# MikeWangWZHL/VidIL

Hardware: AMD Instinct MI355X
Metric: frames/sec whole-node (BLIP caption+filt + CLIP visual-token) 224^2 8f/video (higher is better)
Workload: dtype bf16

## Files before the change

### vidil_amd/csrc/attention.hip

```cpp
#include <type_traits>

#include "common.h"
#include "gemm_epilogue.h"

namespace {

template <typename T>
struct AttnP {
  const T* q;
  const T* k;
  const T* vt;
  T* out;
  const int32_t* kv_len;
  const int32_t* kv_index;
  const int32_t* group_start;
  int Bq, H, Nq, Nk, Tq_cap, Tk_cap, NP, kv_group, causal, causal_off, ldo, n_kv;
  int out_mode;
  int tiled;
  int rb;
  int ostage;
  const float* q32;
  long long ldq32;
  float q_scale;
};
// ... 551 lines not shown
#pragma unroll
      for (int kt = KA - 1; kt < NKT; ++kt) issue_half(uu, kt, 4);
    };
    issue_first(u);
    for (;;) {
      asm volatile("s_waitcnt vmcnt(0)" ::: "memory");
      __builtin_amdgcn_s_barrier();
      issue_second(u);
      asm volatile("s_waitcnt vmcnt(0)" ::: "memory");
      __builtin_amdgcn_s_barrier();
      u += stride;
      if (u >= nunits) break;
      issue_first(u);
    }
    return;
  }

  const int hi = lane >> 5, l31 = lane & 31;
  const int sw = (l31 >> 1) & 7;
  const int row = wave * 32 + l31;
  const bool valid = row < p.Nq;
  const int vc = valid ? row : p.Nq - 1;
  const int vlane = ((lane >> 4) & 1) * VSUB + (hi * 4 + ((lane & 15) >> 2)) * 32 + (lane & 3) * 8;
  char* scratch = smem + NKT * TILE + wave * 2048;
  f16x8 qf[4];
  const uint32_t q_off = (uint32_t)(vc * 128 + hi * 16);
  const __amdgpu_buffer_rsrc_t rsrc_q = uniform_rsrc(p.q, (uint32_t)nunits * p.Tq_cap * 128);
  auto load_q = [&](int uu, f16x8 (&dst)[4]) {
    const uint32_t ub = (uint32_t)uu * p.Tq_cap * 128;
#pragma unroll
    for (int ks = 0; ks < 4; ++ks)
      dst[ks] = __builtin_bit_cast(f16x8, __builtin_amdgcn_raw_buffer_load_b128(rsrc_q, q_off + ks * 32, ub, 0));
  };
  const uint32_t row_off = valid ? (uint32_t)row * p.ldo * (OUT8 ? 1 : 2) : 0x80000000u;
  load_q(u, qf);
  asm volatile("" ::"v"(qf[0]), "v"(qf[1]), "v"(qf[2]), "v"(qf[3]));
  auto read_k2 = [&](int kt, int h2, f16x8 (&kf)[2]) {
    const char* ks_ = smem + kt * TILE + l31 * 128;
#pragma unroll
    for (int j = 0; j < 2; ++j) kf[j] = *(const f16x8*)(ks_ + ((((h2 * 2 + j) * 2 + hi) ^ sw) << 4));
  };
  auto read_v2 = [&](int kt, int hb, f16x8 (&vf)[2]) {
    const char* vs_ = smem + kt * TILE + 4096 + vlane + hb * 512;
#pragma unroll
    for (int dt = 0; dt < 2; ++dt) {
      const char* a = vs_ + dt * (2 * VSUB);
      const s16x4 lo = __builtin_amdgcn_ds_read_tr16_b64_v4i16((__attribute__((address_space(3))) s16x4*)(a));
      const s16x4 hi4 = __builtin_amdgcn_ds_read_tr16_b64_v4i16((__attribute__((address_space(3))) s16x4*)(a + 256));
      typedef short s16x8 __attribute__((ext_vector_type(8)));
      const s16x8 both = __builtin_shufflevector(lo, hi4, 0, 1, 2, 3, 4, 5, 6, 7);
      vf[dt] = __builtin_bit_cast(f16x8, both);
    }
  };
  const f32x16 zero16 = {0.f, 0.f, 0.f, 0.f, 0.f, 0.f, 0.f, 0.f, 0.f, 0.f, 0.f, 0.f, 0.f, 0.f, 0.f, 0.f};
#ifndef VIDIL_ATTN_QAHEAD
#define VIDIL_ATTN_QAHEAD 2
#endif
  constexpr int QAHEAD = VIDIL_ATTN_QAHEAD;
  f16x8 qn[4];
#ifdef VIDIL_ATTN_TIMING
  uint64_t t_b1 = 0, t_b2 = 0, t_st = 0;
  const uint64_t t_begin = __builtin_amdgcn_s_memtime();
#endif
  for (;;) {
    float m, l;
    f32x16 O[2], S;
    f16x8 pf[2];
#ifdef VIDIL_ATTN_TIMING
    const uint64_t tb1 = __builtin_amdgcn_s_memtime();
#endif
    __builtin_amdgcn_s_barrier();
    asm volatile("" ::: "memory");
#ifdef VIDIL_ATTN_TIMING
    t_b1 += __builtin_amdgcn_s_memtime() - tb1;
#endif
    auto fused = [&](int kt, auto first_tag) {
      constexpr bool FIRST = decltype(first_tag)::value;
      f16x8 kf[2], vf[2];
#ifdef VIDIL_ATTN_PRIO
      __builtin_amdgcn_s_setprio(VIDIL_ATTN_PRIO);
#endif
#pragma unroll
      for (int hb = 0; hb < 2; ++hb) {
        read_v2(kt, hb, vf);
        read_k2(kt + 1, hb, kf);
        O[0] = Elt<T>::mfma32(vf[0], pf[hb], FIRST && hb == 0 ? zero16 : O[0]);
        S = Elt<T>::mfma32(kf[0], qf[hb * 2], hb == 0 ? zero16 : S);
        O[1] = Elt<T>::mfma32(vf[1], pf[hb], FIRST && hb == 0 ? zero16 : O[1]);
        S = Elt<T>::mfma32(kf[1], qf[hb * 2 + 1], S);
        __builtin_amdgcn_sched_barrier(0);
      }
#ifdef VIDIL_ATTN_PRIO
      __builtin_amdgcn_s_setprio(0);
#endif
    };
    {
      f16x8 kf[2];
      read_k2(0, 0, kf);
      S = Elt<T>::mfma32(kf[0], qf[0], zero16);
      S = Elt<T>::mfma32(kf[1], qf[1], S);
      read_k2(0, 1, kf);
      S = Elt<T>::mfma32(kf[0], qf[2], S);
      S = Elt<T>::mfma32(kf[1], qf[3], S);
    }
    softmax_tile<T, false, true>(S, 0, nk, false, m, l, O, pf);
    fused(0, std::true_type{});
#pragma unroll 1
    for (int kt = 1; kt < NKT - 1; ++kt) {
      if (kt == QAHEAD) load_q(u + stride < nunits ? u + stride : u, qn);
      softmax_tile<T, false>(S, kt * 32, nk, false, m, l, O, pf);
#ifdef VIDIL_ATTN_TIMING
      const uint64_t tb2 = __builtin_amdgcn_s_memtime();
#endif
      if (kt == KA - 1) __builtin_amdgcn_s_barrier();
      asm volatile("" ::: "memory");
#ifdef VIDIL_ATTN_TIMING
      if (kt == KA - 1) t_b2 += __builtin_amdgcn_s_memtime() - tb2;
#endif
      fused(kt, std::false_type{});
    }
    const int un = u + stride;
    const int bk = u / p.H, h = u - bk * p.H;
#pragma unroll
    for (int ks = 0; ks < 4; ++ks) qf[ks] = qn[ks];
    softmax_tile<T, true>(S, (NKT - 1) * 32, nk, true, m, l, O, pf);
#pragma unroll
    for (int hb = 0; hb < 2; ++hb) {
      f16x8 vf[2];
      read_v2(NKT - 1, hb, vf);
      O[0] = Elt<T>::mfma32(vf[0], pf[hb], O[0]);
      O[1] = Elt<T>::mfma32(vf[1], pf[hb], O[1]);
    }
    l += __shfl_xor(l, 32, 64);
    const float inv = l > 0.f ? 1.0f / l : 0.f;
#ifdef VIDIL_ATTN_TIMING
    const uint64_t ts0 = __builtin_amdgcn_s_memtime();
#endif
#if defined(VIDIL_ATTN_ABLATE) && (VIDIL_ATTN_ABLATE & 2)
    if (inv == 12345.f)
#endif
    {
      if constexpr (OUT8) {
        const __amdgpu_buffer_rsrc_t rsrc = uniform_rsrc((const char*)p.out + ((size_t)bk * p.Nq * p.ldo + h * 64), (uint32_t)p.Nq * p.ldo);
        store_rows_stream_fp8(rsrc, row_off, O, inv, scratch);
      } else {
        const __amdgpu_buffer_rsrc_t rsrc = uniform_rsrc(p.out + ((size_t)bk * p.Nq * p.ldo + h * 64), (uint32_t)p.Nq * p.ldo * 2);
        store_rows_stream<T>(rsrc, row_off, O, inv, scratch);
      }
    }
#ifdef VIDIL_ATTN_TIMING
    t_st += __builtin_amdgcn_s_memtime() - ts0;
#endif
    if (un >= nunits) break;
    u = un;
  }
#ifdef VIDIL_ATTN_TIMING
  if (lane == 0) {
    asm volatile("s_waitcnt vmcnt(0)" ::: "memory");
    uint64_t* dbg = (uint64_t*)p.out + ((size_t)blockIdx.x * 8 + wave) * 4;
    dbg[0] = __builtin_amdgcn_s_memtime() - t_begin;
    dbg[1] = t_b1;
    dbg[2] = t_b2;
    dbg[3] = t_st;
  }
#endif
}

template <typename T, bool QS, int D, bool TILED>
__global__ __launch_bounds__(256, (QS || !TILED) ? 2 : 3) void attn_direct1_kernel(const AttnP<T> p) {
  using f16 = T;
  using f16x8 = typename Elt<T>::x8;
  constexpr int NBUF = D + 1;
  const int lane = threadIdx.x & 63;
  const int wave = __builtin_amdgcn_readfirstlane(threadIdx.x >> 6);
  const int hi = lane >> 5, l31 = lane & 31;
  const int unit = blockIdx.x * 4 + wave;
  if (unit >= p.H * p.n_kv) return;
  const int z = unit / p.H, h = unit - z * p.H;
  int bk, first, count;
  resolve_unit(p, z, bk, first, count);
  const int rows = count * p.Nq;
  if (rows <= 0) return;
  const int nk = p.Nk;
  const RowInfo ri = row_info(p, l31, first, rows);
  const f16* kg = p.k + ((size_t)bk * p.H + h) * p.Tk_cap * 64;
  const f16* vg = p.vt + ((size_t)bk * p.H + h) * 64 * (size_t)(TILED ? p.Tk_cap : p.NP);
  const int ntiles = (nk + 31) >> 5;

  f16x8 kf[NBUF][4], vf[NBUF][2][2];
  auto load = [&](f16x8 (&kfb)[4], f16x8 (&vfb)[2][2], int kt) {
#pragma unroll
    for (int ks = 0; ks < 4; ++ks) kfb[ks] = zero8<T>();
#pragma unroll
    for (int dt = 0; dt < 2; ++dt)
#pragma unroll
      for (int hb = 0; hb < 2; ++hb) vfb[dt][hb] = zero8<T>();
    if constexpr (TILED) {
      const f16* kt_base = kg + (size_t)kt * 2048 + (hi * 32 + l31) * 8;
      if (kt * 32 + l31 < nk) {
#pragma unroll
        for (int ks = 0; ks < 4; ++ks) kfb[ks] = *(const f16x8*)(kt_base + ks * 512);
      }
      const f16* vt_base = vg + (size_t)kt * 2048 + (hi * 32 + l31) * 8;
#pragma unroll
      for (int hb = 0; hb < 2; ++hb) {
        if ((kt * 2 + hb) * 16 + 4 * hi < nk) {
#pragma unroll
          for (int dt = 0; dt < 2; ++dt) vfb[dt][hb] = *(const f16x8*)(vt_base + (hb * 2 + dt) * 512);
        }
      }
    } else {
      int krow = kt * 32 + l31;
      krow = krow < nk ? krow : nk - 1;
      const f16* kr = kg + (size_t)krow * 64 + hi * 8;
#pragma unroll
      for (int ks = 0; ks < 4; ++ks) kfb[ks] = *(const f16x8*)(kr + ks * 16);
#pragma unroll
      for (int hb = 0; hb < 2; ++hb) {
        const int blk0 = (kt * 2 + hb) * 16;
        if (blk0 < nk) {
#pragma unroll
          for (int dt = 0; dt < 2; ++dt) vfb[dt][hb] = *(const f16x8*)(vg + (size_t)(dt * 32 + l31) * p.NP + blk0 + 8 * hi);
        }
      }
    }
  };
#pragma unroll
  for (int j = 0; j < D; ++j)
    if (j < ntiles) load(kf[j], vf[j], j);

  f16x8 qf[4], ql[QS ? 4 : 1];
  if constexpr (QS) {
    const float* qg = p.q32 + ((size_t)ri.qb * p.Nq + ri.t) * p.ldq32 + h * 64 + hi * 8;
#pragma unroll
    for (int ks = 0; ks < 4; ++ks) {
      const f32x4 a = *(const f32x4*)(qg + ks * 16) * p.q_scale, b = *(const f32x4*)(qg + ks * 16 + 4) * p.q_scale;
#pragma unroll
      for (int e = 0; e < 4; ++e) {
        qf[ks][e] = Elt<T>::from_f32(a[e]);
        ql[ks][e] = Elt<T>::from_f32(a[e] - (float)qf[ks][e]);
        qf[ks][4 + e] = Elt<T>::from_f32(b[e]);
        ql[ks][4 + e] = Elt<T>::from_f32(b[e] - (float)qf[ks][4 + e]);
      }
    }
  } else {
    const f16* qg = p.q + (((size_t)ri.qb * p.H + h) * p.Tq_cap + ri.t) * 64 + hi * 8;
#pragma unroll
    for (int ks = 0; ks < 4; ++ks) qf[ks] = *(const f16x8*)(qg + ks * 16);
  }
  int kmin = ri.klim;
#pragma unroll
  for (int o = 32; o > 0; o >>= 1) {
    const int x = __shfl_xor(kmin, o, 64);
    kmin = x < kmin ? x : kmin;
  }
  float m = -INFINITY, l = 0.f;
  f32x16 O[2];
#pragma unroll
  for (int dt = 0; dt < 2; ++dt)
#pragma unroll
    for (int r = 0; r < 16; ++r) O[dt][r] = 0.f;

  auto compute = [&](const f16x8 (&kfb)[4], const f16x8 (&vfb)[2][2], int kt) {
    f32x16 S;
#pragma unroll
    for (int r = 0; r < 16; ++r) S[r] = 0.f;
    if constexpr (QS) {
#pragma unroll
      for (int ks = 0; ks < 4; ++ks) S = Elt<T>::mfma32(kfb[ks], ql[ks], S);
    }
#pragma unroll
    for (int ks = 0; ks < 4; ++ks) S = Elt<T>::mfma32(kfb[ks], qf[ks], S);
    const bool tail = (kt * 32 + 32) > nk;
    const bool need_mask = (kt * 32 + 32) > kmin;
    auto vfrag = [&](int dt, int hb) {
      const int blk0 = (kt * 2 + hb) * 16;
      f16x8 v = vfb[dt][hb];
      if (tail) {
#pragma unroll
        for (int e = 0; e < 8; ++e)
          if (blk0 + 4 * hi + (e & 3) + 8 * (e >> 2) >= nk) v[e] = (f16)0.f;
      }
      return v;
    };
    if constexpr (QS) softmax_pv_tile_psplit<T>(S, kt * 32, ri.klim, need_mask, m, l, O, vfrag);
    else softmax_pv_tile<T, true, false>(S, kt * 32, ri.klim, need_mask, m, l, O, vfrag);
  };
#pragma unroll 1
  for (int kt0 = 0; kt0 < ntiles; kt0 += NBUF) {
#pragma unroll
    for (int j = 0; j < NBUF; ++j) {
      const int kt = kt0 + j;
      if (kt < ntiles) {
        if (kt + D < ntiles) load(kf[(j + D) % NBUF], vf[(j + D) % NBUF], kt + D);
        compute(kf[j], vf[j], kt);
      }
    }
  }
  l += __shfl_xor(l, 32, 64);
  store_rows(p, ri, h, O, l > 0.f ? 1.0f / l : 0.f);
}

template <typename T>
__global__ __launch_bounds__(64) void attn_wave_kernel(const AttnP<T> p) {
  using f16 = T;
  using f16x8 = typename Elt<T>::x8;
  const int lane = threadIdx.x & 63;
  const int hi = lane >> 5, l31 = lane & 31;
  const int h = blockIdx.y;
  int bk, first, count;
  resolve_unit(p, blockIdx.z, bk, first, count);
  const int rows = count * p.Nq;
  if (rows <= 0) return;
  const int nk = p.Nk;
  const RowInfo ri = row_info(p, l31, first, rows);
  const f16* kg = p.k + ((size_t)bk * p.H + h) * p.Tk_cap * 64;
  const f16* vg = p.vt + ((size_t)bk * p.H + h) * 64 * (size_t)p.NP;
  const f16* qg = p.q + (((size_t)ri.qb * p.H + h) * p.Tq_cap + ri.t) * 64 + hi * 8;
  int krow = l31 < nk ? l31 : nk - 1;
  const f16* kr = kg + (size_t)krow * 64 + hi * 8;
  f16x8 kf[4], qf[4], vf[2][2];
#pragma unroll
  for (int ks = 0; ks < 4; ++ks) {
    kf[ks] = *(const f16x8*)(kr + ks * 16);
    qf[ks] = *(const f16x8*)(qg + ks * 16);
  }
#pragma unroll
  for (int dt = 0; dt < 2; ++dt)
#pragma unroll
    for (int hb = 0; hb < 2; ++hb) {
      const int blk0 = hb * 16;
      vf[dt][hb] = zero8<T>();
      if (blk0 < nk) vf[dt][hb] = *(const f16x8*)(vg + (size_t)(dt * 32 + l31) * p.NP + blk0 + 8 * hi);
    }
  f32x16 S;
#pragma unroll
  for (int r = 0; r < 16; ++r) S[r] = 0.f;
#pragma unroll
  for (int ks = 0; ks < 4; ++ks) S = Elt<T>::mfma32(kf[ks], qf[ks], S);
  float m = -INFINITY, l = 0.f;
  f32x16 O[2];
#pragma unroll
  for (int dt = 0; dt < 2; ++dt)
#pragma unroll
    for (int r = 0; r < 16; ++r) O[dt][r] = 0.f;
  softmax_pv_tile<T>(S, 0, ri.klim, true, m, l, O, [&](int dt, int hb) {
    const int blk0 = hb * 16;
    f16x8 v = vf[dt][hb];
#pragma unroll
    for (int e = 0; e < 8; ++e)
      if (blk0 + 4 * hi + (e & 3) + 8 * (e >> 2) >= nk) v[e] = (f16)0.f;
    return v;
  });
  l += __shfl_xor(l, 32, 64);
  store_rows(p, ri, h, O, l > 0.f ? 1.0f / l : 0.f);
}

template <typename T, int NKT, int NW>
int launch_lds(const AttnP<T>& p, int max_rows, hipStream_t s) {
  constexpr int smem_kv = NKT * 32 * KROW * 2 + 64 * (NKT * 32 + 8) * 2;
  constexpr bool ostage = 2 * (smem_kv + NW * 2048) <= 160 * 1024;
  constexpr int smem = smem_kv + (ostage ? NW * 2048 : 0);
  static std::atomic<unsigned long long> attr_set{0};
  auto kern = attn_lds_kernel<T, NKT, NW>;
  if (const int rc_ = vidil_lds_opt_in(attr_set, (const void*)kern, smem, "attention")) return rc_;
  AttnP<T> q = p;
  q.ostage = (ostage && p.ldo % 8 == 0 && ((uintptr_t)p.out & 15) == 0) ? 1 : 0;
  q.rb = (p.Nk <= NKT * 32 && max_rows > NW * 32 && max_rows <= NW * 32 + NW * 16) ? 2 : 1;
  dim3 grid((max_rows + NW * 32 * q.rb - 1) / (NW * 32 * q.rb), p.H, p.n_kv);
  hipLaunchKernelGGL(kern, grid, dim3(NW * 64), smem, s, q);
  VIDIL_CHECK_LAUNCH("attention");
  return VIDIL_OK;
}

template <typename T>
bool stream_eligible(const AttnP<T>& p, int max_rows) {
  const char* e = vidil_dev_env("VIDIL_ATTN_STREAM");
  if (e != nullptr && e[0] == '0') return false;
  return p.NP == 0 && p.kv_len == nullptr && p.kv_index == nullptr && p.group_start == nullptr && p.kv_group == 1 && !p.causal &&
         max_rows > 128 && max_rows <= 224 && p.Nk > 192 && !p.tiled && (p.out_mode == 0 ? p.ldo % 8 == 0 : (p.out_mode == 1 && p.ldo % 16 == 0)) &&
         (uint64_t)p.Nq * p.ldo * 2 < 0x80000000ull && (uint64_t)p.n_kv * p.H * p.Tq_cap * 128 < 0x100000000ull && (((uintptr_t)p.k | (uintptr_t)p.vt | (uintptr_t)p.q | (uintptr_t)p.out) & 15) == 0;
}

template <typename T, int NKT>
int launch_stream(const AttnP<T>& p, hipStream_t s) {
  constexpr int smem = NKT * (4096 + 4 * 1152) + 8 * 2048;
  static_assert(2 * smem <= 160 * 1024, "two workgroups per CU");
  static std::atomic<unsigned long long> attr_set16{0}, attr_set8{0};
  const int n_cu = vidil_cu_count();
  auto kern16 = attn_stream_kernel<T, NKT, false>;
  auto kern8 = attn_stream_kernel<T, NKT, true>;
  if (const int rc_ = vidil_lds_opt_in(attr_set16, (const void*)kern16, smem, "attention (stream kernel)")) return rc_;
  if (const int rc_ = vidil_lds_opt_in(attr_set8, (const void*)kern8, smem, "attention (stream kernel)")) return rc_;
  AttnP<T> q = p;
  q.ostage = 1;
  const int units = p.n_kv * p.H, slots = 2 * n_cu;
  const int rounds = (units + slots - 1) / slots;
  const int grid = (units + rounds - 1) / rounds;
  if (p.out_mode == 1) hipLaunchKernelGGL(kern8, dim3(grid), dim3(512), smem, s, q);
  else hipLaunchKernelGGL(kern16, dim3(grid), dim3(512), smem, s, q);
  VIDIL_CHECK_LAUNCH("attention/stream");
  return VIDIL_OK;
}

template <typename T, bool QS>
int launch_direct1(const AttnP<T>& p, hipStream_t s) {
  VIDIL_REQUIRE((long long)p.H * p.n_kv < 0x7fffffffLL, "attention: H=%d x %d kv batches overflow the unit index", p.H, p.n_kv);
  const int units = p.H * p.n_kv;
  const dim3 grid((units + 3) / 4);
  if (p.tiled) hipLaunchKernelGGL((attn_direct1_kernel<T, QS, 1, true>), grid, dim3(256), 0, s, p);
  else hipLaunchKernelGGL((attn_direct1_kernel<T, QS, 1, false>), grid, dim3(256), 0, s, p);
  VIDIL_CHECK_LAUNCH("attention/direct1");
  return VIDIL_OK;
}

template <typename T, int NKT>
int launch_any(const AttnP<T>& p, int max_rows, hipStream_t s) {
  if constexpr (NKT == 7)
    if (stream_eligible(p, max_rows)) return launch_stream<T, NKT>(p, s);
  if (max_rows <= 32 && NKT == 1 && !p.tiled) {
    hipLaunchKernelGGL(attn_wave_kernel<T>, dim3(1, p.H, p.n_kv), dim3(64), 0, s, p);
    VIDIL_CHECK_LAUNCH("attention/wave");
    return VIDIL_OK;
  }
  if (max_rows <= 32) return launch_direct1<T, false>(p, s);
  if (max_rows > 128) return launch_lds<T, NKT, 8>(p, max_rows, s);
  return launch_lds<T, NKT, 4>(p, max_rows, s);
}

template <typename T>
int attention_dispatch(const AttnP<T>& p, int nkt, int max_rows, int Nk, hipStream_t s) {
  switch (nkt) {
    case 1: return launch_any<T, 1>(p, max_rows, s);
    case 2: return launch_any<T, 2>(p, max_rows, s);
    case 3: return launch_any<T, 3>(p, max_rows, s);
    case 4: return launch_any<T, 4>(p, max_rows, s);
    case 5: return launch_any<T, 5>(p, max_rows, s);
    case 6: return launch_any<T, 6>(p, max_rows, s);
    case 7: return launch_any<T, 7>(p, max_rows, s);
    case 8: return launch_any<T, 8>(p, max_rows, s);
    case 9: return launch_any<T, 9>(p, max_rows, s);
    default: break;
  }
  if (nkt <= 24) {
    if (max_rows <= 32) return launch_direct1<T, false>(p, s);
    if (max_rows > 128) return launch_lds<T, 7, 8>(p, max_rows, s);
    return launch_lds<T, 7, 4>(p, max_rows, s);
  }
  vidil_set_error("attention: Nk=%d > 768 not supported by these kernels", Nk);
  return VIDIL_EUNSUP;
}

}

extern "C" int vidil_attention(const void* q, const void* k, const void* vt, void* out, const int32_t* kv_len,
                               const int32_t* kv_index, const int32_t* group_start, int32_t n_kv, int32_t max_group,
                               int32_t Bq, int32_t H, int32_t Nq, int32_t Nk, int32_t Tq_cap, int32_t Tk_cap, int32_t NP,
                               int32_t kv_group, int32_t causal, int32_t causal_off, int32_t ldo, int32_t kv_tiled,
                               int32_t dtype, int32_t out_dtype, void* stream) {
  VIDIL_REQUIRE(q && k && vt && out, "attention: null pointer");
  VIDIL_REQUIRE(Bq > 0 && H > 0 && Nq > 0 && Nk > 0, "attention: bad shape Bq=%d H=%d Nq=%d Nk=%d", Bq, H, Nq, Nk);
  if (kv_tiled) {
    VIDIL_REQUIRE(Tq_cap >= Nq && Tk_cap >= Nk && Tk_cap % 32 == 0,
                  "attention: tiled K/V need Tk_cap=%d >= Nk=%d and a multiple of 32", Tk_cap, Nk);
    NP = Tk_cap;
  }
  VIDIL_REQUIRE(Tq_cap >= Nq && Tk_cap >= Nk && (NP == 0 || NP >= Nk), "attention: capacities too small");
  VIDIL_REQUIRE(NP % 16 == 0, "attention: NP=%d must be a multiple of 16 (V^T rows hold whole 16-key blocks)", NP);
  VIDIL_REQUIRE(ldo >= H * 64 && ldo % 8 == 0, "attention: ldo=%d must be >= H*64 and a multiple of 8", ldo);
  VIDIL_REQUIRE(kv_group > 0, "attention: kv_group=%d", kv_group);
  int units, max_rows;
  if (group_start != nullptr) {
    VIDIL_REQUIRE(kv_index == nullptr, "attention: group_start and kv_index are mutually exclusive");
    VIDIL_REQUIRE(n_kv > 0 && max_group > 0, "attention: group_start needs n_kv and max_group");
    units = n_kv;
    max_rows = max_group * Nq;
  } else if (kv_index != nullptr) {
    units = Bq;
    max_rows = Nq;
  } else {
    VIDIL_REQUIRE(Bq % kv_group == 0, "attention: Bq=%d not a multiple of kv_group=%d", Bq, kv_group);
    units = Bq / kv_group;
    max_rows = kv_group * Nq;
  }
  VIDIL_REQUIRE(H <= 65535 && units <= 65535, "attention: grid too large (H=%d units=%d)", H, units);
  const int nkt = (Nk + 31) / 32;
  VIDIL_REQUIRE(!kv_tiled || max_rows <= 32, "attention: tiled K/V serve at most 32 query rows per unit (got %d)", max_rows);
  VIDIL_REQUIRE(NP != 0 || max_rows > 32, "attention: row-major V (NP == 0) needs more than 32 query rows per unit (got %d)",
                max_rows);
  const bool split3 = out_dtype == (dtype | VIDIL_DT_SPLIT3);
  VIDIL_REQUIRE(out_dtype == dtype || split3 || (out_dtype == VIDIL_DT_FP8 && max_rows > 32 && ldo % 16 == 0),
                "attention: out_dtype=%d must equal dtype=%d (optionally | VIDIL_DT_SPLIT3), or be fp8 with more than 32 query "
                "rows per unit (staged kernel)", out_dtype, dtype);
  VIDIL_REQUIRE(!split3 || (ldo % 24 == 0 && ldo / 3 >= H * 64), "attention: split3 output needs ldo=%d = 3 planes of >= H*64, "
                "each a multiple of 8", ldo);
  VIDIL_DISPATCH_DTYPE(dtype, "attention", {
    const AttnP<T> p{(const T*)q, (const T*)k, (const T*)vt, (T*)out, kv_len, kv_index, group_start, Bq, H, Nq, Nk,
                     Tq_cap, Tk_cap, NP, kv_group, causal, causal_off, ldo, units, out_dtype == VIDIL_DT_FP8 ? 1 : (split3 ? 2 : 0),
                     kv_tiled ? 1 : 0, 1};
    return attention_dispatch<T>(p, nkt, max_rows, Nk, (hipStream_t)stream);
  });
}

namespace {

struct AttnF32P {
  const float* q;
  const float* k;
  const float* v;
  void* out;
  long long ldq, ldk, ldv, ldo;
  int q_off, k_off, v_off;
  int out_mode;
  int dtype16;
  const int32_t* kv_len;
  const int32_t* kv_index;
  const int32_t* group_start;
  int Bq, H, Nq, Nk, kv_rows, kv_group, causal, causal_off, n_kv;
  const int32_t* anc;
  int anc_ld, arena_rows;
  float scale;
};

template <typename T16>
__device__ __forceinline__ void store_f32_row(const AttnF32P& p, size_t row, int h, int d, float v) {
  if (p.out_mode == 0) {
    ((float*)p.out)[row * p.ldo + h * 64 + d] = v;
  } else {
    const long long pl = p.ldo / 3;
    T16* o = (T16*)p.out + row * p.ldo + h * 64 + d;
    const T16 hi = Elt<T16>::from_f32(v);
    const T16 lo = Elt<T16>::from_f32(v - (float)hi);
    o[0] = hi;
    o[pl] = lo;
    if (p.out_mode != 3) o[2 * pl] = hi;
  }
}

constexpr int F32_KC = 64;
constexpr int F32_LD = 68;
constexpr int F32_RB = 32;

template <typename T16>
__global__ __launch_bounds__(256) void attn_f32_kernel(const AttnF32P p) {
  __shared__ __attribute__((aligned(16))) float Ks[F32_KC * F32_LD];
  __shared__ __attribute__((aligned(16))) float Vs[F32_KC * F32_LD];
  __shared__ __attribute__((aligned(16))) float Qs[F32_RB * F32_LD];
  __shared__ __attribute__((aligned(16))) float Ps[4][4][F32_KC];
  const int tid = threadIdx.x, lane = tid & 63;
  const int wave = __builtin_amdgcn_readfirstlane(tid >> 6);
  const int h = blockIdx.y;
  int bk, first, count;
  resolve_unit(p, blockIdx.z, bk, first, count);
  const int rows = count * p.Nq;
  const int base = blockIdx.x * F32_RB;
  if (base >= rows) return;
  for (int i = tid; i < F32_RB * 16; i += 256) {
    const int r = i >> 4, c = i & 15;
    const RowInfo ri = row_info(p, base + r, first, rows);
    f32x4 qv = {0.f, 0.f, 0.f, 0.f};
    if (ri.valid) qv = *(const f32x4*)(p.q + ((size_t)ri.qb * p.Nq + ri.t) * p.ldq + p.q_off + h * 64 + c * 4);
    *(f32x4*)(Qs + r * F32_LD + c * 4) = qv * p.scale;
  }
  float m[2][4], l[2][4], acc[2][4];
  int klim[2][4];
#pragma unroll
  for (int g = 0; g < 2; ++g)
#pragma unroll
    for (int r = 0; r < 4; ++r) {
      m[g][r] = -INFINITY; l[g][r] = 0.f; acc[g][r] = 0.f;
      const RowInfo ri = row_info(p, base + wave * 8 + g * 4 + r, first, rows);
      klim[g][r] = ri.valid ? ri.klim : 0;
    }
  const float* kg = p.k + (size_t)bk * p.kv_rows * p.ldk + p.k_off + h * 64;
  const float* vg = p.v + (size_t)bk * p.kv_rows * p.ldv + p.v_off + h * 64;
  for (int k0 = 0; k0 < p.Nk; k0 += F32_KC) {
    __syncthreads();
    for (int i = tid; i < F32_KC * 16; i += 256) {
      const int r = i >> 4, c = i & 15;
      f32x4 kv = {0.f, 0.f, 0.f, 0.f}, vv = {0.f, 0.f, 0.f, 0.f};
      if (k0 + r < p.Nk) {
        kv = *(const f32x4*)(kg + (size_t)(k0 + r) * p.ldk + c * 4);
        vv = *(const f32x4*)(vg + (size_t)(k0 + r) * p.ldv + c * 4);
      }
      *(f32x4*)(Ks + r * F32_LD + c * 4) = kv;
      *(f32x4*)(Vs + r * F32_LD + c * 4) = vv;
    }
    __syncthreads();
#pragma unroll
    for (int g = 0; g < 2; ++g) {
      const int kmax = max(max(klim[g][0], klim[g][1]), max(klim[g][2], klim[g][3]));
      if (kmax <= k0) continue;
      float sc[4] = {0.f, 0.f, 0.f, 0.f};
      const float* krow = Ks + lane * F32_LD;
      const float* qrow = Qs + (wave * 8 + g * 4) * F32_LD;
#pragma unroll 4
      for (int c = 0; c < 16; ++c) {
        const f32x4 kv = *(const f32x4*)(krow + c * 4);
#pragma unroll
        for (int r = 0; r < 4; ++r) {
          const f32x4 qv = *(const f32x4*)(qrow + r * F32_LD + c * 4);
          sc[r] = __builtin_fmaf(qv[0], kv[0], sc[r]);
          sc[r] = __builtin_fmaf(qv[1], kv[1], sc[r]);
          sc[r] = __builtin_fmaf(qv[2], kv[2], sc[r]);
          sc[r] = __builtin_fmaf(qv[3], kv[3], sc[r]);
        }
      }
      float alpha[4];
#pragma unroll
      for (int r = 0; r < 4; ++r) {
        const float s = (k0 + lane < klim[g][r]) ? sc[r] : -INFINITY;
        const float mn = fmaxf(m[g][r], wave_max(s));
        const float msafe = mn == -INFINITY ? 0.f : mn;
        const float pr = expf(s - msafe);
        alpha[r] = expf(m[g][r] - msafe);
        l[g][r] = l[g][r] * alpha[r] + wave_sum(pr);
        m[g][r] = mn;
        Ps[wave][r][lane] = pr;
      }
#pragma unroll
      for (int r = 0; r < 4; ++r) acc[g][r] *= alpha[r];
      for (int j = 0; j < F32_KC; j += 4) {
        f32x4 pv[4];
#pragma unroll
        for (int r = 0; r < 4; ++r) pv[r] = *(const f32x4*)(&Ps[wave][r][j]);
#pragma unroll
        for (int e = 0; e < 4; ++e) {
          const float v = Vs[(j + e) * F32_LD + lane];
#pragma unroll
          for (int r = 0; r < 4; ++r) acc[g][r] = __builtin_fmaf(pv[r][e], v, acc[g][r]);
        }
      }
    }
  }
#pragma unroll
  for (int g = 0; g < 2; ++g)
#pragma unroll
    for (int r = 0; r < 4; ++r) {
      const RowInfo ri = row_info(p, base + wave * 8 + g * 4 + r, first, rows);
      if (!ri.valid) continue;
      const float inv = l[g][r] > 0.f ? 1.0f / l[g][r] : 0.f;
      store_f32_row<T16>(p, (size_t)ri.qb * p.Nq + ri.t, h, lane, acc[g][r] * inv);
    }
}

constexpr int F32M_LDK = 68, F32M_LDV = 72;

template <typename T16>
__global__ __launch_bounds__(256) void attn_f32_mfma_kernel(const AttnF32P p) {
  __shared__ __attribute__((aligned(16))) float Ks[32 * F32M_LDK];
  __shared__ __attribute__((aligned(16))) float Vs[32 * F32M_LDV];
  const int tid = threadIdx.x, lane = tid & 63;
  const int wave = __builtin_amdgcn_readfirstlane(tid >> 6);
  const int hi = lane >> 5, l31 = lane & 31;
  const int h = blockIdx.y;
  int bk, first, count;
  resolve_unit(p, blockIdx.z, bk, first, count);
  const int rows = count * p.Nq;
  const int base = blockIdx.x * 128;
  if (base >= rows) return;
  const RowInfo ri = row_info(p, base + wave * 32 + l31, first, rows);
  const bool wave_live = base + wave * 32 < rows;
  float qf[32];
  {
    const float* qrow = p.q + ((size_t)ri.qb * p.Nq + ri.t) * p.ldq + p.q_off + h * 64 + hi * 32;
#pragma unroll
    for (int c = 0; c < 8; ++c) {
      const f32x4 v = *(const f32x4*)(qrow + c * 4);
      qf[c * 4 + 0] = v[0] * p.scale; qf[c * 4 + 1] = v[1] * p.scale; qf[c * 4 + 2] = v[2] * p.scale; qf[c * 4 + 3] = v[3] * p.scale;
    }
  }
  const float* kg = p.k + (size_t)bk * p.kv_rows * p.ldk + p.k_off + h * 64;
  const float* vg = p.v + (size_t)bk * p.kv_rows * p.ldv + p.v_off + h * 64;
  const int skey = tid >> 3, sc = tid & 7;
  f32x4 kr[2], vr[2];
  auto fetch = [&](int k0) {
    const int key = k0 + skey;
#pragma unroll
    for (int j = 0; j < 2; ++j) {
      kr[j] = f32x4{0.f, 0.f, 0.f, 0.f};
      vr[j] = f32x4{0.f, 0.f, 0.f, 0.f};
      if (key < p.Nk) {
        kr[j] = *(const f32x4*)(kg + (size_t)key * p.ldk + (sc + 8 * j) * 4);
        vr[j] = *(const f32x4*)(vg + (size_t)key * p.ldv + (sc + 8 * j) * 4);
      }
    }
  };
  float m = -INFINITY, l = 0.f;
  f32x16 O[2];
#pragma unroll
  for (int dt = 0; dt < 2; ++dt)
#pragma unroll
    for (int r = 0; r < 16; ++r) O[dt][r] = 0.f;
  fetch(0);
  for (int k0 = 0; k0 < p.Nk; k0 += 32) {
    __syncthreads();
#pragma unroll
    for (int j = 0; j < 2; ++j) {
      *(f32x4*)(Ks + skey * F32M_LDK + (sc + 8 * j) * 4) = kr[j];
      *(f32x4*)(Vs + skey * F32M_LDV + (sc + 8 * j) * 4) = vr[j];
    }
    __syncthreads();
    if (k0 + 32 < p.Nk) fetch(k0 + 32);
    if (!wave_live) continue;
    f32x16 S;
#pragma unroll
    for (int r = 0; r < 16; ++r) S[r] = 0.f;
    const float* kp = Ks + l31 * F32M_LDK + hi * 32;
#pragma unroll
    for (int c = 0; c < 8; ++c) {
      const f32x4 kv = *(const f32x4*)(kp + c * 4);
      S = __builtin_amdgcn_mfma_f32_32x32x2f32(kv[0], qf[c * 4 + 0], S, 0, 0, 0);
      S = __builtin_amdgcn_mfma_f32_32x32x2f32(kv[1], qf[c * 4 + 1], S, 0, 0, 0);
      S = __builtin_amdgcn_mfma_f32_32x32x2f32(kv[2], qf[c * 4 + 2], S, 0, 0, 0);
      S = __builtin_amdgcn_mfma_f32_32x32x2f32(kv[3], qf[c * 4 + 3], S, 0, 0, 0);
    }
    float mt = -INFINITY;
#pragma unroll
    for (int r = 0; r < 16; ++r) {
      const int key = k0 + (r & 3) + 8 * (r >> 2) + 4 * hi;
      if (key >= ri.klim) S[r] = -INFINITY;
      mt = fmaxf(mt, S[r]);
    }
    mt = fmaxf(mt, __shfl_xor(mt, 32, 64));
    const float mn = fmaxf(m, mt);
    const float msafe = mn == -INFINITY ? 0.f : mn;
// ... 417 lines not shown
```

Measured before the change: 5082.

## Make small-sequence attention wave kernel persistent with software-pipelined unit loads

The one-wave-per-(head,batch) attention kernel becomes a persistent kernel of four waves per block, with the grid capped at occupancy times CU count. Each wave loops over units with a stride and prefetches the next unit's Q/K/V fragments right after the QK MFMAs, so load latency overlaps the softmax/PV work. Output can also be staged through LDS for coalesced stores. This cuts launch and block-scheduling overhead for many tiny blocks, at the cost of extra register pressure from the double-buffered fragments and a possible load imbalance in the tail.

```diff
diff --git a/vidil_amd/csrc/attention.hip b/vidil_amd/csrc/attention.hip
--- a/vidil_amd/csrc/attention.hip
+++ b/vidil_amd/csrc/attention.hip
@@ -877,58 +877,112 @@
 }
 
 template <typename T>
-__global__ __launch_bounds__(64) void attn_wave_kernel(const AttnP<T> p) {
+__global__ __launch_bounds__(256, 3) void attn_wave_kernel(const AttnP<T> p) {
   using f16 = T;
   using f16x8 = typename Elt<T>::x8;
+  struct Unit {
+    f16x8 kf[4], qf[4], vf[2][2];
+    RowInfo ri;
+    int h, rows;
+  };
+  __shared__ __attribute__((aligned(16))) char scratch[4 * 2048];
   const int lane = threadIdx.x & 63;
   const int hi = lane >> 5, l31 = lane & 31;
-  const int h = blockIdx.y;
-  int bk, first, count;
-  resolve_unit(p, blockIdx.z, bk, first, count);
-  const int rows = count * p.Nq;
-  if (rows <= 0) return;
+  const int wave = __builtin_amdgcn_readfirstlane(threadIdx.x >> 6);
   const int nk = p.Nk;
-  const RowInfo ri = row_info(p, l31, first, rows);
-  const f16* kg = p.k + ((size_t)bk * p.H + h) * p.Tk_cap * 64;
-  const f16* vg = p.vt + ((size_t)bk * p.H + h) * 64 * (size_t)p.NP;
-  const f16* qg = p.q + (((size_t)ri.qb * p.H + h) * p.Tq_cap + ri.t) * 64 + hi * 8;
-  int krow = l31 < nk ? l31 : nk - 1;
-  const f16* kr = kg + (size_t)krow * 64 + hi * 8;
-  f16x8 kf[4], qf[4], vf[2][2];
-#pragma unroll
-  for (int ks = 0; ks < 4; ++ks) {
-    kf[ks] = *(const f16x8*)(kr + ks * 16);
-    qf[ks] = *(const f16x8*)(qg + ks * 16);
-  }
-#pragma unroll
-  for (int dt = 0; dt < 2; ++dt)
-#pragma unroll
-    for (int hb = 0; hb < 2; ++hb) {
+  const int units = p.n_kv * p.H;
+  const int stride = gridDim.x * 4;
+  auto load = [&](int u, Unit& U) {
+    const int z = u / p.H;
+    U.h = u - z * p.H;
+    int bk, first, count;
+    resolve_unit(p, z, bk, first, count);
+    U.rows = count * p.Nq;
+    if (U.rows <= 0) {
+#pragma unroll
+      for (int i = 0; i < 4; ++i) U.kf[i] = U.qf[i] = U.vf[i >> 1][i & 1] = zero8<T>();
+      U.ri = RowInfo{0, 0, 0, false};
+      return;
+    }
+    U.ri = row_info(p, l31, first, U.rows);
+    const f16* kg = p.k + ((size_t)bk * p.H + U.h) * p.Tk_cap * 64;
+    const f16* vg = p.vt + ((size_t)bk * p.H + U.h) * 64 * (size_t)p.NP;
+    const f16* qg = p.q + (((size_t)U.ri.qb * p.H + U.h) * p.Tq_cap + U.ri.t) * 64 + hi * 8;
+    const int krow = l31 < nk ? l31 : nk - 1;
+    const f16* kr = kg + (size_t)krow * 64 + hi * 8;
+#pragma unroll
+    for (int ks = 0; ks < 4; ++ks) {
+      U.kf[ks] = *(const f16x8*)(kr + ks * 16);
+      U.qf[ks] = *(const f16x8*)(qg + ks * 16);
+    }
+#pragma unroll
+    for (int dt = 0; dt < 2; ++dt)
+#pragma unroll
+      for (int hb = 0; hb < 2; ++hb) {
+        const int blk0 = hb * 16 < nk ? hb * 16 : 0;
+        U.vf[dt][hb] = *(const f16x8*)(vg + (size_t)(dt * 32 + l31) * p.NP + blk0 + 8 * hi);
+      }
+  };
+  auto step = [&](const Unit& U, int u, Unit& N) {
+    const int un = u + stride < units ? u + stride : units - 1;
+    if (U.rows <= 0) {
+      load(un, N);
+      return;
+    }
+    f32x16 S;
+#pragma unroll
+    for (int r = 0; r < 16; ++r) S[r] = 0.f;
+#pragma unroll
+    for (int ks = 0; ks < 4; ++ks) S = Elt<T>::mfma32(U.kf[ks], U.qf[ks], S);
+    __builtin_amdgcn_sched_barrier(0);
+    load(un, N);
+    float m = -INFINITY, l = 0.f;
+    f32x16 O[2];
+#pragma unroll
+    for (int dt = 0; dt < 2; ++dt)
+#pragma unroll
+      for (int r = 0; r < 16; ++r) O[dt][r] = 0.f;
+    softmax_pv_tile<T>(S, 0, U.ri.klim, true, m, l, O, [&](int dt, int hb) {
       const int blk0 = hb * 16;
-      vf[dt][hb] = zero8<T>();
-      if (blk0 < nk) vf[dt][hb] = *(const f16x8*)(vg + (size_t)(dt * 32 + l31) * p.NP + blk0 + 8 * hi);
-    }
-  f32x16 S;
-#pragma unroll
-  for (int r = 0; r < 16; ++r) S[r] = 0.f;
-#pragma unroll
-  for (int ks = 0; ks < 4; ++ks) S = Elt<T>::mfma32(kf[ks], qf[ks], S);
-  float m = -INFINITY, l = 0.f;
-  f32x16 O[2];
-#pragma unroll
-  for (int dt = 0; dt < 2; ++dt)
-#pragma unroll
-    for (int r = 0; r < 16; ++r) O[dt][r] = 0.f;
-  softmax_pv_tile<T>(S, 0, ri.klim, true, m, l, O, [&](int dt, int hb) {
-    const int blk0 = hb * 16;
-    f16x8 v = vf[dt][hb];
-#pragma unroll
-    for (int e = 0; e < 8; ++e)
-      if (blk0 + 4 * hi + (e & 3) + 8 * (e >> 2) >= nk) v[e] = (f16)0.f;
-    return v;
-  });
-  l += __shfl_xor(l, 32, 64);
-  store_rows(p, ri, h, O, l > 0.f ? 1.0f / l : 0.f);
+      f16x8 v = U.vf[dt][hb];
+#pragma unroll
+      for (int e = 0; e < 8; ++e)
+        if (blk0 + 4 * hi + (e & 3) + 8 * (e >> 2) >= nk) v[e] = (f16)0.f;
+      return v;
+    });
+    l += __shfl_xor(l, 32, 64);
+    if (p.ostage) store_rows_lds(p, U.ri, U.h, O, l > 0.f ? 1.0f / l : 0.f, scratch + wave * 2048);
+    else store_rows(p, U.ri, U.h, O, l > 0.f ? 1.0f / l : 0.f);
+  };
+  int u = blockIdx.x * 4 + wave;
+  if (u >= units) return;
+  Unit cur;
+  load(u, cur);
+#pragma unroll 1
+  for (; u < units; u += stride) {
+    Unit nxt;
+    step(cur, u, nxt);
+    cur = nxt;
+  }
+}
+
+template <typename T>
+int launch_wave(const AttnP<T>& p, hipStream_t s) {
+  VIDIL_REQUIRE((long long)p.H * p.n_kv < 0x7fffffffLL, "attention: H=%d x %d kv batches overflow the unit index", p.H, p.n_kv);
+  auto kern = attn_wave_kernel<T>;
+  static std::atomic<int> per_cu{0};
+  int wg = per_cu.load();
+  if (wg == 0) {
+    if (hipOccupancyMaxActiveBlocksPerMultiprocessor(&wg, (const void*)kern, 256, 0) != hipSuccess || wg <= 0) wg = 1;
+    per_cu.store(wg);
+  }
+  AttnP<T> q = p;
+  q.ostage = (p.out_mode == 0 && p.ldo % 8 == 0 && ((uintptr_t)p.out & 15) == 0) ? 1 : 0;
+  const int units = p.H * p.n_kv;
+  const int grid = std::min((units + 3) / 4, wg * vidil_cu_count());
+  hipLaunchKernelGGL(kern, dim3(grid), dim3(256), 0, s, q);
+  VIDIL_CHECK_LAUNCH("attention/wave");
+  return VIDIL_OK;
 }
 
 template <typename T, int NKT, int NW>
@@ -994,9 +1048,7 @@
   if constexpr (NKT == 7)
     if (stream_eligible(p, max_rows)) return launch_stream<T, NKT>(p, s);
   if (max_rows <= 32 && NKT == 1 && !p.tiled) {
-    hipLaunchKernelGGL(attn_wave_kernel<T>, dim3(1, p.H, p.n_kv), dim3(64), 0, s, p);
-    VIDIL_CHECK_LAUNCH("attention/wave");
-    return VIDIL_OK;
+    return launch_wave<T>(p, s);
   }
   if (max_rows <= 32) return launch_direct1<T, false>(p, s);
   if (max_rows > 128) return launch_lds<T, NKT, 8>(p, max_rows, s);
```

After: 5089 (median of 5 runs). About the same (+0.1%).
